# ChristianFeldmann/libHM

Hardware: AMD Instinct MI355X
Metric: decoded Mpixels/s (luma), 2160p Main10 reconstruction + loop filters (higher is better)
Workload: dtype int16 samples / int32 accumulate; 1 GPU; 3840x2160 Main10 lowdelay_P pictures, pre-parsed CTU metadata: prep+MC+dequant/IT/recon+deblock+SAO, batch of 16 independent pictures per step, inputs resident in HBM; sub_benchmark=full, streams=2, parallelism=frame-parallel, 1 process per GPU, no data-path collective

## Files before the change

### libhm_amd/csrc/hmgpu_api.hip

```cpp
#include "hmgpu_dev.h"
#include "packed_format.h"

#include <algorithm>
#include <chrono>
#include <atomic>
#include <cstdio>
#include <cstring>
#include <cstdlib>
#include <cmath>
#include <map>
#include <memory>
#include <mutex>
#include <tuple>
#include <new>
#include <thread>
#include <unordered_map>
#include <vector>

using namespace hmgpu;

namespace {

enum { K_PREP = 0, K_MC_LUMA, K_MC_CHROMA, K_ITX, K_DBK_VER, K_DBK_HOR, K_SAO, K_EXTEND, K_H2D, K_INTRA, K_FILTER, K_UNPACK, K_MC_CELLS };
const char* const kKernelNames[HMGPU_NUM_KERNELS] = {"prep", "mc_luma", "mc_chroma", "itx", "deblock_ver", "deblock_hor", "sao",
// ... 386 lines not shown
  return HMGPU_OK;
}

hmgpu_status run_recon(hmgpu_ctx* c, const Batch& b, bool any_intra, bool any_wp, bool any_cells, bool any_bi, bool any_islice) {
  int max_ctus = 0;
  for (int i = 0; i < b.n; i++) max_ctus = std::max(max_ctus, b.num_ctus[i]);
  { ProfScope ps(c, K_PREP); launch_prep(c->d_pics, b, max_ctus, c->parts, any_intra, any_bi, any_cells || c->fmt != 1, c->fmt, c->stream); }
  if (c->fmt != 1) {
    for (int i = 0; i < b.n; i++) {
      const PicDev& d = c->pics[b.pic[i]].dev;
      HIP_TRY(c, hipMemsetAsync(d.resid[1], 0, (size_t)((char*)d.resid[2] - (char*)d.resid[1]) + c->coef_elems[2] * sizeof(int16_t), c->stream));
    }
  }
  McArgs ma;
  memset(&ma, 0, sizeof(ma));
  ma.n = b.n; ma.width = c->seq.width; ma.height = c->seq.height; ma.log2ctu = c->seq.log2_ctu_size; ma.ctus_w = c->ctus_w;
  ma.tw = c->grid_w / 2; ma.npics = c->seq.max_pictures;
  ma.slab = c->plane_slab; ma.pic_stride = 2 * c->plane_bytes; ma.slab_bytes = ma.pic_stride * c->pics.size(); ma.sao_off = (uint32_t)c->plane_bytes;
  for (size_t i = 0; i < c->pics.size(); i++)
    if (c->pics[i].sao_applied) (i < 32 ? ma.sao_mask_lo : ma.sao_mask_hi) |= 1u << (i & 31);
  for (int i = 0; i < b.n; i++) {
    const PicDev& d = c->pics[b.pic[i]].dev;
    ma.first_ctu[i] = b.first_ctu[i]; ma.num_ctus[i] = b.num_ctus[i];
    ma.tmv[i] = d.tmv; ma.slices[i] = d.slices;
  }
  const PicDev& d0 = c->pics[b.pic[0]].dev;
  const char* const base0 = (const char*)c->pics[b.pic[0]].planes;
  uint32_t bps = (uint32_t)std::max(4, std::min(b.n >= 4 ? 12 : 24, max_ctus / 8 + 1));
  {
    ItxArgs ia;
    memset(&ia, 0, sizeof(ia));
    ia.n = b.n; ia.class_mask = 0xf;
    for (int k = 0; k < 3; k++) { ia.rtw[k] = (c->grid_w / 2) >> (k ? c->csx : 0); ia.bd[k] = d0.bd[k]; }
    ia.csx = c->csx; ia.csy = c->csy;
    for (int k = 0; k < 4; k++) ia.tu_cap[k] = c->tu_cap[k];
    for (int i = 0; i < b.n; i++) {
      const PicDev& d = c->pics[b.pic[i]].dev;
      for (int k = 0; k < 4; k++) ia.tu[i][k] = d.tu[k];
      ia.tu_count[i] = d.tu_count;
      for (int k = 0; k < 3; k++) { ia.coef[i][k] = d.coef[k]; ia.resid[i][k] = d.resid[k]; }
      ia.sl_m[i] = d.sl_m;
    }
    ProfScope ps(c, K_ITX);
    launch_itx(ia, bps, c->stream);
    bool any_ccp = false;
    for (int i = 0; i < b.n; i++) any_ccp |= c->pics[b.pic[i]].dev.ccp[0] != nullptr;
    if (any_ccp) launch_ccp(c->d_pics, b, max_ctus, c->stream);
  }
  {
    ProfScope ps(c, K_MC_LUMA);
    ma.pitch = c->pitch[0]; ma.bd = c->seq.bit_depth_luma;
    ma.origin_off = (uint32_t)((const char*)d0.rec[0] - base0);
    ma.rtw = c->grid_w / 2;
    for (int i = 0; i < b.n; i++) { ma.dst[i] = c->pics[b.pic[i]].dev.rec[0]; ma.resid[i] = c->pics[b.pic[i]].dev.resid[0]; }
    launch_mc_luma(ma, max_ctus, any_wp, any_bi, c->stream);
    if (any_cells) { ProfScope pc(c, K_MC_CELLS); launch_mc_luma_cells(c->d_pics, c->d_finals, b, max_ctus, c->seq.log2_ctu_size, any_wp, c->stream); }
  }
  if (c->fmt != 1) {
    ProfScope ps(c, K_MC_CHROMA);
    launch_mc_chroma_fmt(c->d_pics, c->d_finals, b, max_ctus, c->seq.log2_ctu_size, c->fmt, any_wp, c->stream);
  } else if (c->seq.chroma_format != 0) {
    ProfScope ps(c, K_MC_CHROMA);
    ma.pitch = c->pitch[1]; ma.bd = c->seq.bit_depth_chroma;
    ma.origin_off = (uint32_t)((const char*)d0.rec[1] - base0);
    ma.cr_off = 0;
    ma.rtw = c->grid_w / 4;
    for (int i = 0; i < b.n; i++) {
      const PicDev& d = c->pics[b.pic[i]].dev;
      ma.dst[i] = d.rec[1]; ma.dst2[i] = d.rec[2]; ma.resid[i] = d.resid[1]; ma.resid2[i] = d.resid[2];
    }
    launch_mc_chroma(ma, max_ctus, any_wp, any_bi, c->stream);
    if (any_cells) { ProfScope pc(c, K_MC_CELLS); launch_mc_chroma_cells(c->d_pics, c->d_finals, b, max_ctus, c->seq.log2_ctu_size, any_wp, c->stream); }
  }
  if (any_intra) {
    ProfScope ps(c, K_INTRA);
    launch_intra(c->d_pics, b, c->d_ctu_order, c->num_ctus, !any_islice, c->stream);
    if (c->fmt == 2) launch_intra_chroma_422(c->d_pics, b, c->stream);
    for (int i = 0; i < b.n; i++) if (std::find(c->intra_launched.begin(), c->intra_launched.end(), b.pic[i]) == c->intra_launched.end()) c->intra_launched.push_back(b.pic[i]);
  }
  HIP_TRY(c, hipGetLastError());
  return HMGPU_OK;
}

hmgpu_status run_filter(hmgpu_ctx* c, const Batch& b, int stages) {
  bool all_sao = stages == 7 && c->fmt == 1;
  for (int i = 0; i < b.n && all_sao; i++) all_sao = c->pics[b.pic[i]].sao_any;
  if (all_sao) {
    bool nofilt = false;
    for (int i = 0; i < b.n; i++) nofilt |= c->pics[b.pic[i]].dev.any_nofilt != 0;
    { ProfScope ps(c, K_FILTER); launch_filter_fused(c->d_pics, b, c->seq.width, c->seq.height, nofilt, c->stream); }
    HIP_TRY(c, hipGetLastError());
    return HMGPU_OK;
  }
  if (stages & 1) { ProfScope ps(c, K_DBK_VER); launch_deblock(c->d_pics, b, 0, c->seq.width, c->seq.height, c->stream);
                    if (c->fmt != 1) launch_deblock_chroma_fmt(c->d_pics, b, 0, c->seq.width, c->seq.height, c->stream); }
  if (stages & 2) { ProfScope ps(c, K_DBK_HOR); launch_deblock(c->d_pics, b, 1, c->seq.width, c->seq.height, c->stream);
                    if (c->fmt != 1) launch_deblock_chroma_fmt(c->d_pics, b, 1, c->seq.width, c->seq.height, c->stream); }
  if (stages & 4) {
    bool any = false;
    for (int i = 0; i < b.n; i++) any |= c->pics[b.pic[i]].sao_any;
    if (any) { ProfScope ps(c, K_SAO); launch_sao(c->d_pics, b, c->seq.width, c->seq.height, c->csx, c->csy, c->stream); }
  }
  HIP_TRY(c, hipGetLastError());
  return HMGPU_OK;
}

hmgpu_status stage_sao(hmgpu_ctx* c, Picture& p, const hmgpu_pic_params* pp, const hmgpu_sao_param* sao,
                       const std::vector<uint16_t>& slice_idx, const std::vector<uint16_t>& tile_idx) {
  const int n = c->num_ctus;
  std::vector<const hmgpu_sao_param*> res((size_t)n * 3);
  std::vector<SaoDev>& dev = p.h_saoprm;
  dev.resize((size_t)n * 3);
  bool any = false;
  for (int a = 0; a < n; a++) {
    const int cx = a % c->ctus_w, cy = a / c->ctus_w;
    const hmgpu_sao_param* const* merge[2] = {nullptr, nullptr};
    auto same = [&](int o) { return slice_idx[o] == slice_idx[a] && tile_idx[o] == tile_idx[a]; };
    if (cx > 0 && same(a - 1)) merge[HMGPU_SAO_MERGE_LEFT] = &res[(size_t)(a - 1) * 3];
    if (cy > 0 && same(a - c->ctus_w)) merge[HMGPU_SAO_MERGE_ABOVE] = &res[(size_t)(a - c->ctus_w) * 3];
    unsigned avail = 1u << 4;
    for (int k = 0; k < 9; k++) {
      if (k == 4) continue;
      const int nx = cx + k % 3 - 1, ny = cy + k / 3 - 1;
      if (nx < 0 || nx >= c->ctus_w || ny < 0 || ny >= c->ctus_h) continue;
      const int o = ny * c->ctus_w + nx;
      bool ok = true;
      if (slice_idx[o] != slice_idx[a]) {
        const SliceDev& later = p.slices[std::max(slice_idx[o], slice_idx[a])];
        ok = later.lf_across_slices != 0;
      }
      if (ok && !pp->lf_across_tiles) ok = tile_idx[o] == tile_idx[a];
      if (ok) avail |= 1u << k;
    }
    for (int comp = 0; comp < 3; comp++) {
      const hmgpu_sao_param* r = &sao[(size_t)a * 3 + comp];
      if (r->mode_idc == HMGPU_SAO_MERGE) {
        if (r->type_idc < 0 || r->type_idc > 1 || !merge[r->type_idc]) return HMGPU_EINVAL;
        r = merge[r->type_idc][comp];
      }
      res[(size_t)a * 3 + comp] = r;
      const int shift = comp == 0 ? pp->sao_offset_shift_luma : pp->sao_offset_shift_chroma;
      SaoDev& d = dev[(size_t)a * 3 + comp];
      memset(&d, 0, sizeof(d));
      d.type = r->mode_idc == HMGPU_SAO_OFF ? -1 : (int8_t)r->type_idc;
      d.avail = (uint16_t)avail;
      if (d.type == HMGPU_SAO_BO) {
        d.band = (uint8_t)(r->type_aux_info & 31);
        for (int i = 0; i < 4; i++) d.off[i] = (int8_t)(r->offset[(r->type_aux_info + i) & 31] * (1 << shift));
      } else if (d.type >= 0) {
        for (int i = 0; i < 5; i++) d.off[i] = (int8_t)(r->offset[i] * (1 << shift));
      }
      any |= d.type >= 0;
    }
  }
  p.sao_any = any;
  HIP_TRY(c, h2d_small(c, p.dev.saoprm, dev.data(), dev.size() * sizeof(SaoDev), c->stream));
  return HMGPU_OK;
}

}

extern "C" {

const char* hmgpu_status_string(hmgpu_status s) {
  switch (s) {
    case HMGPU_OK: return "ok";
    case HMGPU_EINVAL: return "invalid argument";
    case HMGPU_EDEVICE: return "device (HIP) error";
    case HMGPU_EUNSUPPORTED: return "coding tool not supported";
    case HMGPU_ENOMEM: return "out of memory";
  }
  return "?";
}
const char* hmgpu_kernel_name(int32_t k) { return (k >= 0 && k < HMGPU_NUM_KERNELS) ? kKernelNames[k] : ""; }
// ... 1991 lines not shown
  std::vector<std::vector<int>> all(n);
  {
    ProfScope ps(c, K_H2D);
    for (int i = 0; i < n && st == HMGPU_OK; i++) {
      const hmgpu_packed_job& j = jobs[i];
      Picture& p = c->pics[j.pic];
      const hipStream_t hs = (i & 1) ? c->copy_stream2 : c->copy_stream;
      wait_for_last_use(c, p, hs);
      if (p.sao_applied) { p.sao_applied = false; p.dev.sao_applied = 0; for (int k = 0; k < 3; k++) c->h_finals[j.pic].p[k] = p.dev.rec[k];
                           HIP_TRY(c, h2d_small(c, c->d_finals + j.pic, &c->h_finals[j.pic], sizeof(PlaneSet), hs)); }
      bool wp = false;
      { HostTimer ts(c, 1);
      for (int k = 0; k < j.num_slices && st == HMGPU_OK; k++) {
        st = register_slice(c, j.pic, k, j.slices[k], hs);
        all[i].push_back(k);
        wp |= j.slices[k] && j.slices[k]->weighted_pred != 0;
      }
      }
      SliceCall call;
      HostTimer ti(c, 2);
      if (st == HMGPU_OK) st = stage_packed(c, j, sums[i], all[i], wp, hs, &call);
      if (st != HMGPU_OK) break;
      b.pic[i] = j.pic; b.first_ctu[i] = 0; b.num_ctus[i] = c->num_ctus;
      ua.pic[i] = j.pic; ua.blob[i] = (const char*)p.blob;
      any_intra |= call.intra; any_wp |= call.wp; any_cells |= call.cells; any_bi |= call.bi; any_islice |= call.islice;
    }
    if (n > 1) {
      (void)hipEventRecord(c->copy_join, c->copy_stream2);
      (void)hipStreamWaitEvent(c->copy_stream, c->copy_join, 0);
    }
    if (st != HMGPU_OK) return st;
    c->copy_seq++;
    if (c->copy_seq > 8 && hipEventQuery(c->copy_ev[(c->copy_seq - 7) % 8]) == hipSuccess)
      for (auto it = c->packed_reads.begin(); it != c->packed_reads.end();) it = it->second <= c->copy_seq - 7 ? c->packed_reads.erase(it) : std::next(it);
    for (int i = 0; i < n; i++) c->packed_reads[jobs[i].blob] = c->copy_seq;
    HIP_TRY(c, hipEventRecord(c->copy_ev[c->copy_seq % 8], c->copy_stream));
    HIP_TRY(c, hipStreamWaitEvent(c->stream, c->copy_ev[c->copy_seq % 8], 0));
  }
  HostTimer tr(c, 3);
  { ProfScope ps(c, K_UNPACK); launch_unpack_input(c->d_pics, ua, c->num_ctus, c->stream); }
  HIP_TRY(c, hipGetLastError());
  for (int i = 0; i < n && st == HMGPU_OK; i++) st = extend_refs_of(c, jobs[i].pic, all[i]);
  if (st == HMGPU_OK) st = run_recon(c, b, any_intra, any_wp, any_cells, any_bi, any_islice);
  mark_use(c, b);
  return st;
}

hmgpu_status hmgpu_packed_wait(hmgpu_ctx* c, const void* blob) {
  if (!c || !blob) return HMGPU_EINVAL;
  const auto it = c->packed_reads.find(blob);
  if (it == c->packed_reads.end()) return HMGPU_OK;
  hipSetDevice(c->device);
  const uint64_t seq = c->copy_seq - it->second < 8 ? it->second : c->copy_seq;
  if (hipEventSynchronize(c->copy_ev[seq % 8]) != hipSuccess) return HMGPU_EDEVICE;
  return HMGPU_OK;
}

hmgpu_status hmgpu_filter_pictures(hmgpu_ctx* c, int32_t n, const hmgpu_filter_job* jobs) {
  if (!c || !jobs || n < 1 || n > kMaxBatch) return HMGPU_EINVAL;
  for (int i = 0; i < n; i++) {
    if (!valid_pic(c, jobs[i].pic) || !jobs[i].pp) return HMGPU_EINVAL;
    if (jobs[i].pp->sao_enabled && !jobs[i].sao) return HMGPU_EINVAL;
    for (int k = 0; k < i; k++) if (jobs[k].pic == jobs[i].pic) return HMGPU_EINVAL;
  }
  hipSetDevice(c->device);
  Batch b; memset(&b, 0, sizeof(b));
  b.n = n;
  { HostTimer tsao(c, 4);
  for (int i = 0; i < n; i++) {
    Picture& p = c->pics[jobs[i].pic];
    p.sao_any = false;
    if (jobs[i].pp->sao_enabled) {
      std::vector<uint16_t> sidx = p.h_slice_idx, tidx = p.h_tile_idx;
      sidx.resize(c->num_ctus, 0);
      tidx.resize(c->num_ctus, 0);
      hmgpu_status st = stage_sao(c, p, jobs[i].pp, jobs[i].sao, sidx, tidx);
      if (st != HMGPU_OK) return st;
    }
    p.filter_ready = true;
    b.pic[i] = jobs[i].pic; b.first_ctu[i] = 0; b.num_ctus[i] = c->num_ctus;
  }
  }
  HostTimer tf(c, 5);
  hmgpu_status st = run_filter(c, b, 7);
  if (st != HMGPU_OK) return st;
  for (int i = 0; i < n && st == HMGPU_OK; i++) {
    Picture& p = c->pics[jobs[i].pic];
    if (p.sao_any) {
      p.sao_applied = true; p.dev.sao_applied = 1;
      st = push_final(c, jobs[i].pic);
      if (st == HMGPU_OK) st = push_picdev(c, jobs[i].pic);
    }
    p.extended = true;
  }
  if (st != HMGPU_OK) return st;
  { ProfScope ps(c, K_EXTEND); launch_extend(c->d_pics, b, c->seq.width, c->seq.height, c->mx[0], c->my[0], c->csx, c->csy, c->stream); }
  HIP_TRY(c, hipGetLastError());
  mark_use(c, b);
  return HMGPU_OK;
}

hmgpu_status hmgpu_filter_picture_stages(hmgpu_ctx* c, hmgpu_pic cur, const hmgpu_pic_params* pp, const hmgpu_sao_param* sao,
                                         int32_t stages) {
  if (!c || !valid_pic(c, cur) || !pp) return HMGPU_EINVAL;
  if ((stages & 4) && pp->sao_enabled && !sao) return HMGPU_EINVAL;
  hipSetDevice(c->device);
  Picture& p = c->pics[cur];
  p.sao_any = false;
  if ((stages & 4) && pp->sao_enabled) {
    std::vector<uint16_t> sidx = p.h_slice_idx, tidx = p.h_tile_idx;
    sidx.resize(c->num_ctus, 0);
    tidx.resize(c->num_ctus, 0);
    hmgpu_status st = stage_sao(c, p, pp, sao, sidx, tidx);
    if (st != HMGPU_OK) return st;
  }
  p.filter_ready = true;
  Batch b; memset(&b, 0, sizeof(b));
  b.n = 1; b.pic[0] = cur; b.first_ctu[0] = 0; b.num_ctus[0] = c->num_ctus;
  hmgpu_status st = run_filter(c, b, stages);
  if (st != HMGPU_OK) return st;
  if ((stages & 4) && p.sao_any) {
    p.sao_applied = true; p.dev.sao_applied = 1;
    st = push_final(c, cur);
    if (st == HMGPU_OK) st = push_picdev(c, cur);
    if (st != HMGPU_OK) return st;
  }
  p.extended = false;
  st = ensure_extended(c, cur);
  commit_use(c);
  return st;
}

hmgpu_status hmgpu_filter_picture(hmgpu_ctx* c, hmgpu_pic cur, const hmgpu_pic_params* pp, const hmgpu_sao_param* sao) {
  return hmgpu_filter_picture_stages(c, cur, pp, sao, 7);
}

hmgpu_status hmgpu_replay_batch(hmgpu_ctx* c, const hmgpu_pic* pics, int32_t n, int32_t stages, int32_t iters) {
  if (!c || !pics || n < 1 || n > kMaxBatch || iters < 0) return HMGPU_EINVAL;
  size_t ncalls = 0;
  for (int i = 0; i < n; i++) {
    if (!valid_pic(c, pics[i])) return HMGPU_EINVAL;
    if (i == 0) ncalls = c->pics[pics[i]].calls.size();
    else if (c->pics[pics[i]].calls.size() != ncalls) return HMGPU_EINVAL;
  }
  if ((stages & 8) && ncalls == 0) return HMGPU_EINVAL;
  hipSetDevice(c->device);
  const int lanes = (c->replay_streams == 2 && n >= 2 && !c->profiling) ? 2 : 1;
  hipStream_t const main_stream = c->stream;
  if (lanes == 2) {
    HIP_TRY(c, hipEventRecord(c->lane_ev[0], main_stream));
    HIP_TRY(c, hipStreamWaitEvent(c->stream2, c->lane_ev[0], 0));
  }
  hmgpu_status result = HMGPU_OK;
  for (int it = 0; it < iters && result == HMGPU_OK; it++) {
    for (int lane = 0; lane < lanes && result == HMGPU_OK; lane++) {
      const int lo = lanes == 2 ? (lane == 0 ? 0 : n / 2) : 0, hi = lanes == 2 ? (lane == 0 ? n / 2 : n) : n;
      c->stream = lane == 0 ? main_stream : c->stream2;
      if (stages & 8) {
        for (size_t k = 0; k < ncalls && result == HMGPU_OK; k++) {
          Batch b; memset(&b, 0, sizeof(b));
          b.n = hi - lo;
          bool any_intra = false, any_wp = false, any_cells = false, any_bi = false, any_islice = false;
          for (int i = lo; i < hi; i++) {
            const SliceCall& sc = c->pics[pics[i]].calls[k];
            b.pic[i - lo] = pics[i]; b.first_ctu[i - lo] = sc.first_ctu; b.num_ctus[i - lo] = sc.num_ctus;
            any_intra |= sc.intra; any_wp |= sc.wp; any_cells |= sc.cells; any_bi |= sc.bi; any_islice |= sc.islice;
          }
          result = ensure_refs_extended(c, b, k);
          if (result == HMGPU_OK) result = run_recon(c, b, any_intra, any_wp, any_cells, any_bi, any_islice);
        }
      }
      if ((stages & 7) && result == HMGPU_OK) {
        Batch b; memset(&b, 0, sizeof(b));
        b.n = hi - lo;
        for (int i = lo; i < hi; i++) { b.pic[i - lo] = pics[i]; b.first_ctu[i - lo] = 0; b.num_ctus[i - lo] = c->num_ctus; }
        result = run_filter(c, b, stages & 7);
        if (result == HMGPU_OK) {
          { ProfScope ps(c, K_EXTEND); launch_extend(c->d_pics, b, c->seq.width, c->seq.height, c->mx[0], c->my[0], c->csx, c->csy, c->stream); }
          if (hipGetLastError() != hipSuccess) result = HMGPU_EDEVICE;
        }
      }
    }
  }
  c->stream = main_stream;
  if (lanes == 2) {
    HIP_TRY(c, hipEventRecord(c->lane_ev[1], c->stream2));
    HIP_TRY(c, hipStreamWaitEvent(main_stream, c->lane_ev[1], 0));
  }
  for (int i = 0; i < n; i++) touch(c, pics[i]);
  commit_use(c);
  return result;
}

hmgpu_status hmgpu_set_streams(hmgpu_ctx* c, int32_t n) {
  if (!c || n < 1 || n > 2) return HMGPU_EINVAL;
  c->replay_streams = n;
  return HMGPU_OK;
}

hmgpu_status hmgpu_replay(hmgpu_ctx* c, hmgpu_pic cur, int32_t stages, int32_t iters) { return hmgpu_replay_batch(c, &cur, 1, stages, iters); }

hmgpu_status hmgpu_set_profiling(hmgpu_ctx* c, int32_t enable) {
  if (!c) return HMGPU_EINVAL;
  HIP_TRY(c, hipStreamSynchronize(c->stream));
  prof_drain(c);
  c->profiling = enable != 0;
  return HMGPU_OK;
}

hmgpu_status hmgpu_get_stats(hmgpu_ctx* c, hmgpu_stats* out, int32_t reset) {
  if (!c || !out) return HMGPU_EINVAL;
  HIP_TRY(c, hipStreamSynchronize(c->stream));
  prof_drain(c);
  memset(out, 0, sizeof(*out));
  for (int k = 0; k < HMGPU_NUM_KERNELS; k++) { out->kernel_ms[k] = c->kernel_ms[k]; out->kernel_launches[k] = c->kernel_launches[k]; }
  for (Picture& p : c->pics) {
    if (!p.in_use) continue;
    unsigned long long st[2 * kTuShards];
    HIP_TRY(c, hipMemcpy(st, p.dev.stats, sizeof(st), hipMemcpyDeviceToHost));
    for (int s = 0; s < kTuShards; s++) { out->intra_partitions += st[s]; out->inter_partitions += st[kTuShards + s]; }
    if (reset) HIP_TRY(c, hipMemset(p.dev.stats, 0, sizeof(st)));
  }
  if (reset) for (int k = 0; k < HMGPU_NUM_KERNELS; k++) { c->kernel_ms[k] = 0; c->kernel_launches[k] = 0; }
  return HMGPU_OK;
}

hmgpu_status hmgpu_inverse_transform_batch(hmgpu_ctx* c, int32_t log2_size, int32_t bit_depth, int32_t n, const int16_t* levels,
                                           const int8_t* qp_per, const int8_t* qp_rem, const uint8_t* flags, int16_t* resid) {
  if (!c || log2_size < 2 || log2_size > 5 || n < 1 || !levels || !qp_per || !qp_rem || !flags || !resid) return HMGPU_EINVAL;
  if (bit_depth < 8 || bit_depth > 12) return HMGPU_EUNSUPPORTED;
  hipSetDevice(c->device);
  const size_t elems = (size_t)n << (2 * log2_size);
  int16_t *d_lev = nullptr, *d_res = nullptr; int8_t *d_per = nullptr, *d_rem = nullptr; uint8_t* d_fl = nullptr;
  hmgpu_status st = HMGPU_OK;
  auto fail = [&](hipError_t e) { if (e != hipSuccess && st == HMGPU_OK) { c->last_err = (int32_t)e; st = HMGPU_EDEVICE; } };
  fail(hipMalloc((void**)&d_lev, elems * 2)); fail(hipMalloc((void**)&d_res, elems * 2));
  fail(hipMalloc((void**)&d_per, n)); fail(hipMalloc((void**)&d_rem, n)); fail(hipMalloc((void**)&d_fl, n));
  if (st == HMGPU_OK) {
    fail(hipMemcpy(d_lev, levels, elems * 2, hipMemcpyHostToDevice));
    fail(hipMemcpy(d_per, qp_per, n, hipMemcpyHostToDevice)); fail(hipMemcpy(d_rem, qp_rem, n, hipMemcpyHostToDevice));
    fail(hipMemcpy(d_fl, flags, n, hipMemcpyHostToDevice));
  }
  if (st == HMGPU_OK) {
    launch_itx_flat(log2_size, bit_depth, n, d_lev, d_per, d_rem, d_fl, d_res, c->stream);
    fail(hipGetLastError());
    fail(hipStreamSynchronize(c->stream));
    fail(hipMemcpy(resid, d_res, elems * 2, hipMemcpyDeviceToHost));
  }
  hipFree(d_lev); hipFree(d_res); hipFree(d_per); hipFree(d_rem); hipFree(d_fl);
  return st;
}

hmgpu_status hmgpu_mc_batch(hmgpu_ctx* c, int32_t is_chroma, int32_t bit_depth, const int16_t* ref_plane, int32_t ref_stride,
                            int32_t ref_w, int32_t ref_h, int32_t n, const int32_t* blocks, int32_t bi, int16_t* dst) {
  if (!c || !ref_plane || !blocks || !dst || n < 1 || ref_w < 1 || ref_h < 1 || ref_stride < ref_w) return HMGPU_EINVAL;
  if (bit_depth < 8 || bit_depth > 12) return HMGPU_EUNSUPPORTED;
  hipSetDevice(c->device);
  std::vector<int32_t> off(n);
  size_t total = 0;
  for (int i = 0; i < n; i++) {
// ... 40 lines not shown
```

### libhm_amd/csrc/k_filter.hip

```cpp
#include "hmgpu_dev.h"
#include "filter_core.h"
#include <type_traits>

namespace hmgpu {

namespace {
constexpr int kTW = 64, kTH = 64;
constexpr int kYC = kTW + 16, kYH = kTH + 8;
constexpr int kCC = kTW / 2 + 16, kCH = kTH / 2 + 4;
constexpr int kYW = kYC + 8, kCW = kCC + 8;

constexpr int kUnits = 9 * 18;
struct FilterLds {
  __attribute__((aligned(16))) int16_t y[kYH][kYW];
  __attribute__((aligned(16))) int16_t c[2][kCH][kCW];
  uint32_t unit[2][3][64];
  int32_t units[2][4];
};

struct SliceLf { int tc_off, beta_off, cb_off, cr_off; };
struct FPic {
  static constexpr int csx = 1, csy = 1;
  int width, height, bd0, bd1, bd2, log2ctu, ctus_w, pitch[2], grid_w, any_nofilt, mono;
  __device__ inline int bd(int comp) const { return comp == 0 ? bd0 : comp == 1 ? bd1 : bd2; }
// ... 106 lines not shown

template <bool NF>
__device__ inline uint32_t edge_classify(uint32_t rec, uint32_t slice, int u) {
  const uint32_t bs = rec & 3u, qp = (rec >> 2) & 127u;
  const uint32_t p_nf = NF ? (rec >> 9) & 1u : 0u, q_nf = NF ? (rec >> 10) & 1u : 0u;
  const uint32_t e = (uint32_t)u | (bs << 8) | (p_nf << 10) | (q_nf << 11) | ((qp + 32u) << 12) | (slice << 20);
  return bs ? e : 0u;
}

__device__ inline void push_units(uint32_t (&list)[3][64], int32_t (&count)[4], uint32_t rec, int t) {
  const unsigned long long m = __ballot(rec != 0u);
  const int wave = t >> 6, lane = t & 63;
  if (rec != 0u) list[wave][__popcll(m & ((1ull << lane) - 1ull))] = rec;
  if (lane == 0) count[wave] = __popcll(m);
}
__device__ inline uint32_t pop_unit(const uint32_t (&list)[3][64], const int32_t (&count)[4], int t) {
  const int c0 = count[0], c1 = count[1], c2 = count[2];
  if (t < c0) return list[0][t];
  if (t < c0 + c1) return list[1][t - c0];
  if (t < c0 + c1 + c2) return list[2][t - c0 - c1];
  return 0u;
}

template <int DIR, bool NF>
__device__ inline void edge_apply(const FPic& P, FilterLds& L, int x0, int y0, uint32_t rec) {
  if (rec == 0u) return;
  const int u = rec & 0xff, bs = (rec >> 8) & 3, qp = (int)((rec >> 12) & 0xff) - 64, slice = rec >> 20;
  const bool p_nf = NF && ((rec >> 10) & 1), q_nf = NF && ((rec >> 11) & 1);
  const int x = DIR == 0 ? x0 + 8 * (u % 9) : x0 - 4 + 4 * (u % 18);
  const int y = DIR == 0 ? y0 - 4 + 4 * (u / 9) : y0 + 8 * (u / 18);
  const SliceLf sl = slice == 0 ? P.s0 : slice_lf(P.slices + slice);
  const int tc_off = sl.tc_off, beta_off = sl.beta_off;
  int16_t* base = &L.y[y - (y0 - 4)][x - (x0 - 8)];
  uint32_t a[8], b[8];
  if (DIR == 0) {
    uint32_t r[4][4];
#pragma unroll
    for (int i = 0; i < 4; i++) {
      const u32x2 lo = *reinterpret_cast<const u32x2*>(base + i * kYW - 4), hi = *reinterpret_cast<const u32x2*>(base + i * kYW);
      r[i][0] = lo.x; r[i][1] = lo.y; r[i][2] = hi.x; r[i][3] = hi.y;
    }
    rows_to_pairs(r[0], r[1], a);
    rows_to_pairs(r[2], r[3], b);
  } else {
#pragma unroll
    for (int k = 0; k < 8; k++) {
      const u32x2 v = *reinterpret_cast<const u32x2*>(base + (k - 4) * kYW);
      a[k] = v.x; b[k] = v.y;
    }
  }
  filter_luma_unit(a, b, bs, qp, tc_off, beta_off, P.bd(0), p_nf, q_nf);
  if (DIR == 0) {
    uint32_t r[4][4];
    pairs_to_rows(a, r[0], r[1]);
    pairs_to_rows(b, r[2], r[3]);
#pragma unroll
    for (int i = 0; i < 4; i++) {
      *reinterpret_cast<u32x2*>(base + i * kYW - 4) = (u32x2){r[i][0], r[i][1]};
      *reinterpret_cast<u32x2*>(base + i * kYW) = (u32x2){r[i][2], r[i][3]};
    }
  } else {
#pragma unroll
    for (int k = 1; k < 7; k++) *reinterpret_cast<u32x2*>(base + (k - 4) * kYW) = (u32x2){a[k], b[k]};
  }
  if (bs == 2 && ((DIR == 0 ? x : y) & 15) == 0 && !P.mono) {
    const int maxc = (1 << P.bd(1)) - 1;
#pragma unroll
    for (int comp = 1; comp < 3; comp++) {
      const int tc = chroma_tc(qp, comp == 1 ? sl.cb_off : sl.cr_off, tc_off, P.bd(comp));
      int16_t* cb = &L.c[comp - 1][(y >> 1) - ((y0 >> 1) - 2)][(x >> 1) - ((x0 >> 1) - 8)];
#pragma unroll
      for (int i = 0; i < 2; i++) {
        int16_t* s = DIR == 0 ? cb + i * kCW : cb + i;
        const int o = DIR == 0 ? 1 : kCW;
        const int m2 = (uint16_t)s[-2 * o], m3 = (uint16_t)s[-o], m4 = (uint16_t)s[0], m5 = (uint16_t)s[o];
        const int delta = clip3(-tc, tc, ((((m4 - m3) << 2) + m2 - m5 + 4) >> 3));
        if (!p_nf) s[-o] = (int16_t)clip3(0, maxc, m3 + delta);
        if (!q_nf) s[0] = (int16_t)clip3(0, maxc, m4 - delta);
      }
    }
  }
}

}

template <bool NF>
__global__ void __launch_bounds__(256) k_filter_fused(const PicDev* __restrict__ pics, Batch b, int tiles_x, int tiles) {
  __shared__ FilterLds L;
  int slot, lb;
  if (!xcd_remap(blockIdx.x, b.n, tiles, slot, lb)) return;
  const FPic P = pic_state(pics + b.pic[slot]);
  __builtin_amdgcn_sched_barrier(0);
  const int x0 = (lb % tiles_x) * kTW, y0 = (lb / tiles_x) * kTH;
  const int t = threadIdx.x;
  const int l2 = P.log2ctu, p0 = P.pitch[0], p1 = P.pitch[1];
  const int vx = x0 + 8 * (t % 9), vy = y0 - 4 + 4 * (t / 9), hx = x0 - 4 + 4 * (t % 18), hy = y0 + 8 * (t / 18);
  const bool vin = t < kUnits && vy >= 0 && vx < P.width && vy < P.height, hin = t < kUnits && hx >= 0 && hx < P.width && hy < P.height;
  const int ecw = P.grid_w >> 1, ex0 = (x0 >> 3) - 1, ey0 = (y0 >> 3) - 1;
  const Span se(reinterpret_cast<const char*>(P.edges) + ((ptrdiff_t)ey0 * ecw + ex0) * (ptrdiff_t)sizeof(EdgeRec), (uint32_t)((9 * ecw + 10) * (int)sizeof(EdgeRec)));
  const uint32_t ev = se.load_u16(se.at(vin, (uint32_t)((((vy >> 3) - ey0) * ecw + (vx >> 3) - ex0) * 8 + ((vy >> 2) & 1) * 2)));
  const uint32_t eh = se.load_u16(se.at(hin, (uint32_t)((((hy >> 3) - ey0) * ecw + (hx >> 3) - ex0) * 8 + 4 + ((hx >> 2) & 1) * 2)));
  const int sx0 = (x0 - 8) >> l2, sy0 = (y0 - 8) >> l2;
  const Span ss(reinterpret_cast<const char*>(P.slice_idx) + ((ptrdiff_t)sy0 * P.ctus_w + sx0) * 2,
                P.slice_idx ? (uint32_t)(((((y0 + 64) >> l2) - sy0) * P.ctus_w + ((x0 + 64) >> l2) - sx0 + 1) * 2) : 0u);
  uint32_t sv = ss.load_u16(ss.at(vin, (uint32_t)((((vy >> l2) - sy0) * P.ctus_w + (vx >> l2) - sx0) * 2)));
  uint32_t sh = ss.load_u16(ss.at(hin, (uint32_t)((((hy >> l2) - sy0) * P.ctus_w + (hx >> l2) - sx0) * 2)));
  constexpr int VPR = kYC / 8, VPC = 2 * kCC / 8;
  static_assert(kYH * VPR > 512 && kYH * VPR <= 768 && kCH * VPC > 256 && kCH * VPC <= 512, "three rounds of luma vectors, two of chroma");
  const int yr0 = t / VPR, yv0 = t % VPR, yr1 = (t + 256) / VPR, yv1 = (t + 256) % VPR, yr2 = (t + 512) / VPR, yv2 = (t + 512) % VPR;
  const int ur0 = t / VPC, uv0 = t % VPC, ur1 = (t + 256) / VPC, uv1 = (t + 256) % VPC;
  const bool yin2 = t + 512 < kYH * VPR, uin1 = t + 256 < kCH * VPC;
  const Span sy(P.rec[0] + ((ptrdiff_t)(y0 - 4) * p0 + (x0 - 8)), (uint32_t)(((kYH - 1) * p0 + kYC) * 2));
  const Span sc(P.rec[1] + ((ptrdiff_t)((y0 >> 1) - 2) * p1 + kCStep * ((x0 >> 1) - 8)), (uint32_t)(((kCH - 1) * p1 + kCStep * kCC) * 2));
  const u32x4 ty0 = sy.load4((uint32_t)((yr0 * p0 + 8 * yv0) * 2));
  const u32x4 ty1 = sy.load4((uint32_t)((yr1 * p0 + 8 * yv1) * 2));
  const u32x4 ty2 = sy.load4(sy.at(yin2, (uint32_t)((yr2 * p0 + 8 * yv2) * 2)));
  const u32x4 tc0 = sc.load4((uint32_t)((ur0 * p1 + 8 * uv0) * 2));
  const u32x4 tc1 = sc.load4(sc.at(uin1, (uint32_t)((ur1 * p1 + 8 * uv1) * 2)));
  const int gx = (t & 7) * 8, gy = t >> 3;
  const int lx = x0 + gx, ly[2] = {y0 + gy, y0 + gy + 32};
  const int ccomp = 1 + (t & 1), ccx = (x0 >> 1) + ((t >> 1) & 3) * 8, ccy = (y0 >> 1) + gy;
  const bool lin[2] = {lx < P.width && ly[0] < P.height, lx < P.width && ly[1] < P.height}, cin = ccx < (P.width >> 1) && ccy < (P.height >> 1);
  const int n64 = 63 >> l2;
  const Span sp(P.saoprm + ((ptrdiff_t)(y0 >> l2) * P.ctus_w + (x0 >> l2)) * 3, (uint32_t)(((n64 * P.ctus_w + n64) * 3 + 3) * (int)sizeof(SaoDev)));
  const uint32_t prow = (uint32_t)(3 * (int)sizeof(SaoDev)) * (uint32_t)P.ctus_w;
  const SaoPrm sl0 = sao_fetch(sp, sp.at(lin[0], (uint32_t)(gy >> l2) * prow + (uint32_t)((gx >> l2) * 3 * (int)sizeof(SaoDev))));
  const SaoPrm sl1 = sao_fetch(sp, sp.at(lin[1], (uint32_t)((gy + 32) >> l2) * prow + (uint32_t)((gx >> l2) * 3 * (int)sizeof(SaoDev))));
  const SaoPrm sc0 = sao_fetch(sp, sp.at(cin, (uint32_t)((2 * gy) >> l2) * prow + (uint32_t)(((((t >> 1) & 3) * 16) >> l2) * 3 + ccomp) * (uint32_t)sizeof(SaoDev)));
  asm volatile("" : "+v"(sv), "+v"(sh));
  if (t < 192) {
    push_units(L.unit[0], L.units[0], edge_classify<NF>(ev, sv, t), t);
    push_units(L.unit[1], L.units[1], edge_classify<NF>(eh, sh, t), t);
  }
  *reinterpret_cast<u32x4*>(&L.y[yr0][8 * yv0]) = ty0;
  *reinterpret_cast<u32x4*>(&L.y[yr1][8 * yv1]) = ty1;
  if (yin2) *reinterpret_cast<u32x4*>(&L.y[yr2][8 * yv2]) = ty2;
  auto put_chroma = [&](int r, int v, const u32x4 c) {
    *reinterpret_cast<u32x2*>(&L.c[0][r][4 * v]) = u32x2{__builtin_amdgcn_perm(c.y, c.x, 0x05040100u), __builtin_amdgcn_perm(c.w, c.z, 0x05040100u)};
    *reinterpret_cast<u32x2*>(&L.c[1][r][4 * v]) = u32x2{__builtin_amdgcn_perm(c.y, c.x, 0x07060302u), __builtin_amdgcn_perm(c.w, c.z, 0x07060302u)};
  };
  put_chroma(ur0, uv0, tc0);
  if (uin1) put_chroma(ur1, uv1, tc1);
  __syncthreads();
  edge_apply<0, NF>(P, L, x0, y0, pop_unit(L.unit[0], L.units[0], t));
  __syncthreads();
  edge_apply<1, NF>(P, L, x0, y0, pop_unit(L.unit[1], L.units[1], t));
  __syncthreads();
  const Span oy(P.sao[0] + ((ptrdiff_t)y0 * p0 + x0), (uint32_t)(((kTH - 1) * p0 + kTW) * 2));
  if (lin[0]) oy.store4((uint32_t)((gy * p0 + gx) * 2), sao_group<kYW, NF>(P, 0, L.y, x0 - 8, y0 - 4, lx, ly[0], sl0));
  if (lin[1]) oy.store4((uint32_t)(((gy + 32) * p0 + gx) * 2), sao_group<kYW, NF>(P, 0, L.y, x0 - 8, y0 - 4, lx, ly[1], sl1));
  if (cin) {
    const u32x4 own = sao_group<kCW, NF>(P, ccomp, L.c[ccomp - 1], (x0 >> 1) - 8, (y0 >> 1) - 2, ccx, ccy, sc0);
    const bool odd = t & 1;
    const uint32_t r0 = (uint32_t)__shfl_xor((int)(odd ? own.x : own.z), 1, 64), r1 = (uint32_t)__shfl_xor((int)(odd ? own.y : own.w), 1, 64);
    const uint32_t cb0 = odd ? r0 : own.x, cb1 = odd ? r1 : own.y, cr0 = odd ? own.z : r0, cr1 = odd ? own.w : r1;
    const u32x4 o = {__builtin_amdgcn_perm(cr0, cb0, 0x05040100u), __builtin_amdgcn_perm(cr0, cb0, 0x07060302u),
                     __builtin_amdgcn_perm(cr1, cb1, 0x05040100u), __builtin_amdgcn_perm(cr1, cb1, 0x07060302u)};
    const Span oc(P.sao[1] + ((ptrdiff_t)(y0 >> 1) * p1 + kCStep * (x0 >> 1)), (uint32_t)(((kTH / 2 - 1) * p1 + kCStep * kTW / 2) * 2));
    oc.store4((uint32_t)((gy * p1 + kCStep * (((t >> 1) & 3) * 8 + (odd ? 4 : 0))) * 2), o);
  }
}

void launch_filter_fused(const PicDev* pics, const Batch& b, int width, int height, bool nofilt, hipStream_t s) {
  const int tiles_x = (width + kTW - 1) / kTW, tiles = tiles_x * ((height + kTH - 1) / kTH);
  dim3 grid((unsigned)xcd_grid(b.n, tiles));
  if (nofilt) hipLaunchKernelGGL(k_filter_fused<true>, grid, dim3(256), 0, s, pics, b, tiles_x, tiles);
  else hipLaunchKernelGGL(k_filter_fused<false>, grid, dim3(256), 0, s, pics, b, tiles_x, tiles);
}

}
```

Baseline: 195,700 Mpixels/s.

## Fuse picture border extension into the fused deblock+SAO filter kernel

Border tiles of the fused filter kernel now write their SAO output back into LDS and replicate edge samples into the picture margins for luma and interleaved chroma. The host then skips the separate extend kernel whenever the fused path ran. This removes one kernel launch and a separate pass over the border memory for each batch. In exchange, border tiles do extra synchronisation and margin stores, and the host-side bookkeeping of the extended flag becomes more involved.

```diff
diff --git a/libhm_amd/csrc/hmgpu_api.hip b/libhm_amd/csrc/hmgpu_api.hip
--- a/libhm_amd/csrc/hmgpu_api.hip
+++ b/libhm_amd/csrc/hmgpu_api.hip
@@ -492,7 +492,8 @@
   return HMGPU_OK;
 }
 
-hmgpu_status run_filter(hmgpu_ctx* c, const Batch& b, int stages) {
+hmgpu_status run_filter(hmgpu_ctx* c, const Batch& b, int stages, bool* fused) {
+  *fused = false;
   bool all_sao = stages == 7 && c->fmt == 1;
   for (int i = 0; i < b.n && all_sao; i++) all_sao = c->pics[b.pic[i]].sao_any;
   if (all_sao) {
@@ -500,6 +501,7 @@
     for (int i = 0; i < b.n; i++) nofilt |= c->pics[b.pic[i]].dev.any_nofilt != 0;
     { ProfScope ps(c, K_FILTER); launch_filter_fused(c->d_pics, b, c->seq.width, c->seq.height, nofilt, c->stream); }
     HIP_TRY(c, hipGetLastError());
+    *fused = true;
     return HMGPU_OK;
   }
   if (stages & 1) { ProfScope ps(c, K_DBK_VER); launch_deblock(c->d_pics, b, 0, c->seq.width, c->seq.height, c->stream);
@@ -2657,7 +2659,8 @@
   }
   }
   HostTimer tf(c, 5);
-  hmgpu_status st = run_filter(c, b, 7);
+  bool fused;
+  hmgpu_status st = run_filter(c, b, 7, &fused);
   if (st != HMGPU_OK) return st;
   for (int i = 0; i < n && st == HMGPU_OK; i++) {
     Picture& p = c->pics[jobs[i].pic];
@@ -2669,8 +2672,10 @@
     p.extended = true;
   }
   if (st != HMGPU_OK) return st;
-  { ProfScope ps(c, K_EXTEND); launch_extend(c->d_pics, b, c->seq.width, c->seq.height, c->mx[0], c->my[0], c->csx, c->csy, c->stream); }
-  HIP_TRY(c, hipGetLastError());
+  if (!fused) {
+    { ProfScope ps(c, K_EXTEND); launch_extend(c->d_pics, b, c->seq.width, c->seq.height, c->mx[0], c->my[0], c->csx, c->csy, c->stream); }
+    HIP_TRY(c, hipGetLastError());
+  }
   mark_use(c, b);
   return HMGPU_OK;
 }
@@ -2692,7 +2697,8 @@
   p.filter_ready = true;
   Batch b; memset(&b, 0, sizeof(b));
   b.n = 1; b.pic[0] = cur; b.first_ctu[0] = 0; b.num_ctus[0] = c->num_ctus;
-  hmgpu_status st = run_filter(c, b, stages);
+  bool fused;
+  hmgpu_status st = run_filter(c, b, stages, &fused);
   if (st != HMGPU_OK) return st;
   if ((stages & 4) && p.sao_any) {
     p.sao_applied = true; p.dev.sao_applied = 1;
@@ -2700,7 +2706,7 @@
     if (st == HMGPU_OK) st = push_picdev(c, cur);
     if (st != HMGPU_OK) return st;
   }
-  p.extended = false;
+  p.extended = fused;
   st = ensure_extended(c, cur);
   commit_use(c);
   return st;
@@ -2749,8 +2755,12 @@
         Batch b; memset(&b, 0, sizeof(b));
         b.n = hi - lo;
         for (int i = lo; i < hi; i++) { b.pic[i - lo] = pics[i]; b.first_ctu[i - lo] = 0; b.num_ctus[i - lo] = c->num_ctus; }
-        result = run_filter(c, b, stages & 7);
-        if (result == HMGPU_OK) {
+        bool fused = false;
+        result = run_filter(c, b, stages & 7, &fused);
+        for (int i = lo; i < hi && fused; i++) fused = c->pics[pics[i]].sao_applied;
+        if (result == HMGPU_OK && fused) {
+          for (int i = lo; i < hi; i++) c->pics[pics[i]].extended = true;
+        } else if (result == HMGPU_OK) {
           { ProfScope ps(c, K_EXTEND); launch_extend(c->d_pics, b, c->seq.width, c->seq.height, c->mx[0], c->my[0], c->csx, c->csy, c->stream); }
           if (hipGetLastError() != hipSuccess) result = HMGPU_EDEVICE;
         }
diff --git a/libhm_amd/csrc/k_filter.hip b/libhm_amd/csrc/k_filter.hip
--- a/libhm_amd/csrc/k_filter.hip
+++ b/libhm_amd/csrc/k_filter.hip
@@ -212,6 +212,28 @@
   }
 }
 
+template <int E, typename FE, typename FR>
+__device__ inline void tile_margins(int16_t* pl, int pitch, int x0, int xe, int y0, int ye, int w, int h, int mx, int my, int t, FE edge, FR row) {
+  constexpr int VE = 8 / E;
+  const bool left = x0 == 0, right = xe == w, top = y0 == 0, bottom = ye == h;
+  const int ra = top ? -my : y0, rb = bottom ? h + my : ye;
+  const int ca = left ? -mx : x0, cb = right ? w + mx : xe;
+  const Span sm(pl + ((ptrdiff_t)ra * pitch + E * ca), (uint32_t)(((rb - ra - 1) * pitch + E * (cb - ca)) * 2));
+  const unsigned sv = (unsigned)(mx / VE), nside = (left ? sv : 0u) + (right ? sv : 0u);
+  for (unsigned i = (unsigned)t; i < nside * (unsigned)(rb - ra); i += 256u) {
+    const int r = (int)(i / nside), k = (int)(i % nside) - (left ? (int)sv : 0);
+    const int x = k >= 0 ? w + k * VE : k * VE;
+    const uint32_t v = edge(clip3(y0, ye - 1, ra + r), k >= 0 ? w - 1 : 0);
+    sm.store4((uint32_t)((r * pitch + E * (x - ca)) * 2), u32x4{v, v, v, v});
+  }
+  const unsigned tv = (unsigned)((xe - x0) / VE), nband = (top ? (unsigned)my : 0u) + (bottom ? (unsigned)my : 0u);
+  for (unsigned i = (unsigned)t; i < tv * nband; i += 256u) {
+    const int r = (int)(i / tv) - (top ? my : 0), x = x0 + (int)(i % tv) * VE;
+    const int y = r >= 0 ? h + r : r;
+    sm.store4((uint32_t)(((y - ra) * pitch + E * (x - ca)) * 2), row(r >= 0 ? h - 1 : 0, x));
+  }
+}
+
 }
 
 template <bool NF>
@@ -219,7 +241,8 @@
   __shared__ FilterLds L;
   int slot, lb;
   if (!xcd_remap(blockIdx.x, b.n, tiles, slot, lb)) return;
-  const FPic P = pic_state(pics + b.pic[slot]);
+  const PicDev* const pic = pics + b.pic[slot];
+  const FPic P = pic_state(pic);
   __builtin_amdgcn_sched_barrier(0);
   const int x0 = (lb % tiles_x) * kTW, y0 = (lb / tiles_x) * kTH;
   const int t = threadIdx.x;
@@ -277,10 +300,11 @@
   edge_apply<1, NF>(P, L, x0, y0, pop_unit(L.unit[1], L.units[1], t));
   __syncthreads();
   const Span oy(P.sao[0] + ((ptrdiff_t)y0 * p0 + x0), (uint32_t)(((kTH - 1) * p0 + kTW) * 2));
-  if (lin[0]) oy.store4((uint32_t)((gy * p0 + gx) * 2), sao_group<kYW, NF>(P, 0, L.y, x0 - 8, y0 - 4, lx, ly[0], sl0));
-  if (lin[1]) oy.store4((uint32_t)(((gy + 32) * p0 + gx) * 2), sao_group<kYW, NF>(P, 0, L.y, x0 - 8, y0 - 4, lx, ly[1], sl1));
+  u32x4 o0 = {}, o1 = {}, own = {};
+  if (lin[0]) { o0 = sao_group<kYW, NF>(P, 0, L.y, x0 - 8, y0 - 4, lx, ly[0], sl0); oy.store4((uint32_t)((gy * p0 + gx) * 2), o0); }
+  if (lin[1]) { o1 = sao_group<kYW, NF>(P, 0, L.y, x0 - 8, y0 - 4, lx, ly[1], sl1); oy.store4((uint32_t)(((gy + 32) * p0 + gx) * 2), o1); }
   if (cin) {
-    const u32x4 own = sao_group<kCW, NF>(P, ccomp, L.c[ccomp - 1], (x0 >> 1) - 8, (y0 >> 1) - 2, ccx, ccy, sc0);
+    own = sao_group<kCW, NF>(P, ccomp, L.c[ccomp - 1], (x0 >> 1) - 8, (y0 >> 1) - 2, ccx, ccy, sc0);
     const bool odd = t & 1;
     const uint32_t r0 = (uint32_t)__shfl_xor((int)(odd ? own.x : own.z), 1, 64), r1 = (uint32_t)__shfl_xor((int)(odd ? own.y : own.w), 1, 64);
     const uint32_t cb0 = odd ? r0 : own.x, cb1 = odd ? r1 : own.y, cr0 = odd ? own.z : r0, cr1 = odd ? own.w : r1;
@@ -289,6 +313,25 @@
     const Span oc(P.sao[1] + ((ptrdiff_t)(y0 >> 1) * p1 + kCStep * (x0 >> 1)), (uint32_t)(((kTH / 2 - 1) * p1 + kCStep * kTW / 2) * 2));
     oc.store4((uint32_t)((gy * p1 + kCStep * (((t >> 1) & 3) * 8 + (odd ? 4 : 0))) * 2), o);
   }
+  const int xe = min(x0 + kTW, P.width), ye = min(y0 + kTH, P.height);
+  if (x0 != 0 && y0 != 0 && xe != P.width && ye != P.height) return;
+  const int mx0 = ldc(&pic->mx[0]), my0 = ldc(&pic->my[0]), mx1 = ldc(&pic->mx[1]), my1 = ldc(&pic->my[1]);
+  __syncthreads();
+  if (lin[0]) *reinterpret_cast<u32x4*>(&L.y[gy + 4][gx + 8]) = o0;
+  if (lin[1]) *reinterpret_cast<u32x4*>(&L.y[gy + 36][gx + 8]) = o1;
+  if (cin) *reinterpret_cast<u32x4*>(&L.c[ccomp - 1][gy + 2][((t >> 1) & 3) * 8 + 8]) = own;
+  __syncthreads();
+  tile_margins<1>(P.sao[0], p0, x0, xe, y0, ye, P.width, P.height, mx0, my0, t,
+                  [&](int y, int x) { return (uint32_t)(uint16_t)L.y[y - y0 + 4][x - x0 + 8] * 0x10001u; },
+                  [&](int y, int x) { return *reinterpret_cast<const u32x4*>(&L.y[y - y0 + 4][x - x0 + 8]); });
+  const int cx0 = x0 >> 1, cy0 = y0 >> 1;
+  tile_margins<kCStep>(P.sao[1], p1, cx0, xe >> 1, cy0, ye >> 1, P.width >> 1, P.height >> 1, mx1, my1, t,
+                       [&](int y, int x) { return (uint32_t)(uint16_t)L.c[0][y - cy0 + 2][x - cx0 + 8] | (uint32_t)(uint16_t)L.c[1][y - cy0 + 2][x - cx0 + 8] << 16; },
+                       [&](int y, int x) {
+                         const u32x2 cb = *reinterpret_cast<const u32x2*>(&L.c[0][y - cy0 + 2][x - cx0 + 8]), cr = *reinterpret_cast<const u32x2*>(&L.c[1][y - cy0 + 2][x - cx0 + 8]);
+                         return u32x4{__builtin_amdgcn_perm(cr.x, cb.x, 0x05040100u), __builtin_amdgcn_perm(cr.x, cb.x, 0x07060302u),
+                                      __builtin_amdgcn_perm(cr.y, cb.y, 0x05040100u), __builtin_amdgcn_perm(cr.y, cb.y, 0x07060302u)};
+                       });
 }
 
 void launch_filter_fused(const PicDev* pics, const Batch& b, int width, int height, bool nofilt, hipStream_t s) {
```

New measurement: 193,600 Mpixels/s. 0.989x the previous value.
